# NjuHaoZhang/AMMCNet_AAAI2021

Measured on AMD Instinct MI355X. Metric: frames/sec, 256x256x4 dual-stream clips (twostream forward, inference), higher is better.
Workload: dtype f32-equivalent: (hi,lo) f16 split, 3 fp16 MFMAs per product (v_mfma_f32_32x32x16_f16 in the 4-wave k-half-major kernels, 16x16x32 in the 8-wave / fused-decoder kernels), f32 accumulate; 1 GPU; Ped2 full dual-stream + 2000-slot memory module, batch=16, inference (BASELINE.json configs[1]); batch_per_gpu=16, frame=256x256, n_embed=2000, embed_dim=64, k=2, parallelism=replicas x1 (no collective)

## Files before the change

ammcnet_aaai2021_amd/csrc/conv_outc_s16.hip:

```cpp
#include "ammc_common.h"
#include <hip/hip_fp16.h>
#include <stdio.h>
#include <stdlib.h>

namespace ammc_s16 {

typedef _Float16 f16x8o __attribute__((ext_vector_type(8)));

constexpr float O_LO_INV = 1.f / 2048.f;
constexpr int O_TH = 8, O_TW = 32, O_HW = O_TW + 2, O_HP = (O_TH + 2) * O_HW;
constexpr int O_APIECES = O_HP * 8;
constexpr int O_NT = 512;
constexpr int O_R = (O_APIECES + O_NT - 1) / O_NT;
constexpr int O_ASTAGE = ((O_APIECES + 63) / 64) * 64 * 4;
constexpr int O_MAXNS = 4;
constexpr int O_TG = O_MAXNS * 256;
constexpr int O_NS = 3;
constexpr int O_MAXCC = 2;
static_assert(O_R == 6, "OUTC_WAIT below knows 0, 2, 6 and 8 outstanding operations");

struct OutcArgs {
  AmmcConvDesc d;
  int tiles_x, tiles_y, ncc, kpad, total, nstore;
};

#define OUTC_WAIT(n)                                                              \
  switch (n) {                                                                    \
    case 0: asm volatile("s_waitcnt vmcnt(0)" ::: "memory"); break;               \
    case 2: asm volatile("s_waitcnt vmcnt(2)" ::: "memory"); break;               \
    case 6: asm volatile("s_waitcnt vmcnt(6)" ::: "memory"); break;               \
    default: asm volatile("s_waitcnt vmcnt(8)" ::: "memory"); break;              \
  }

__global__ __launch_bounds__(O_NT, 1) void conv_outc_s16_kernel(OutcArgs a) {
  extern __shared__ __attribute__((aligned(16))) float smem[];
  float* As = smem;
  float* Fs = smem + O_NS * O_ASTAGE;
  float* Tg = Fs + 9 * O_MAXCC * 128;
  float* Scr = Tg + 2 * O_TG;
  float* Sq = Scr + 256;

  const int tid = threadIdx.x, lane = tid & 63, wave = tid >> 6;
  const int l15 = lane & 15, g4 = lane >> 4;
  const AmmcConvDesc& d = a.d;
  const int G = gridDim.x;
  const int first = ammc_xcd_remap(blockIdx.x, G);
  const int ntile = (a.total - first + G - 1) / G;
  const int U = ntile * a.ncc;

  for (int i = tid; i < 9 * a.ncc * 32; i += O_NT) {
    const int chunk = i >> 5, row = (i >> 3) & 3, q = i & 7;
    int sl = q ^ row;
    sl ^= (sl >> 1) & 1;
    const f32x4 w = *reinterpret_cast<const f32x4*>(d.w + (int64_t)row * a.kpad + chunk * 32 + 4 * sl);
    *reinterpret_cast<f32x4*>(Fs + chunk * 128 + row * 32 + 4 * q) = w;
  }

  const int ns = a.nstore;
  const int64_t ycs = d.y_cs > 0 ? d.y_cs : 1;
  const bool score = d.sq_target != nullptr;

  float sc = 1.f, sh = 0.f;
  if (g4 < ns) {
    if (d.scale) sc = d.scale[g4];
    if (d.shift) sh = d.shift[g4];
  }
  asm volatile("" : "+v"(sc), "+v"(sh));

  int a_off[O_R];
#pragma unroll
  for (int j = 0; j < O_R; ++j) {
    int p = j * O_NT + tid;
    p = p < O_APIECES ? p : O_APIECES - 1;
    const int hp = p >> 3;
    int ls = (p & 7) ^ (hp & 7);
    ls ^= (ls >> 1) & 1;
    const int hy = hp / O_HW;
    const int hx = hp - hy * O_HW;
    a_off[j] = (int)((int64_t)hy * d.x_rs + (int64_t)hx * d.x_ps) + 4 * ls;
  }
#define OUTC_ISSUE(tile_, cc_, stage_)                                                                            \
  {                                                                                                               \
    int sp_ = (tile_);                                                                                            \
    const int tx_ = sp_ % a.tiles_x;                                                                              \
    sp_ /= a.tiles_x;                                                                                             \
    const int ty_ = sp_ % a.tiles_y;                                                                              \
    const int b_ = sp_ / a.tiles_y;                                                                               \
    const float* xp_ = d.x + ((int64_t)b_ * d.x_bs + (int64_t)(ty_ * O_TH) * d.x_rs + (int64_t)(tx_ * O_TW) * d.x_ps) + (cc_) * 32; \
    float* dst_ = As + (stage_) * O_ASTAGE + wave * 256;                                                          \
    _Pragma("unroll") for (int j = 0; j < O_R; ++j)                                                               \
      __builtin_amdgcn_global_load_lds(xp_ + a_off[j], (j * O_NT + wave * 64) * 4 < O_ASTAGE ? dst_ + j * O_NT * 4 : Scr, 16, 0, 0); \
  }
  const int tg_e0 = tid < ns * 256 ? tid : 0, tg_e1 = 512 + tid < ns * 256 ? 512 + tid : 0;
  const int64_t tg_o0 = (tg_e0 >> 8) * ycs + ((tg_e0 >> 5) & 7) * d.y_rs + (tg_e0 & 31) * d.y_ps;
  const int64_t tg_o1 = (tg_e1 >> 8) * ycs + ((tg_e1 >> 5) & 7) * d.y_rs + (tg_e1 & 31) * d.y_ps;
#define OUTC_ISSUE_TG(tile_, buf_)                                                                                \
  {                                                                                                               \
    int sp_ = (tile_);                                                                                            \
    const int tx_ = sp_ % a.tiles_x;                                                                              \
    sp_ /= a.tiles_x;                                                                                             \
    const int ty_ = sp_ % a.tiles_y;                                                                              \
    const int b_ = sp_ / a.tiles_y;                                                                               \
    const float* tp_ = d.sq_target + ((int64_t)b_ * d.y_bs + (int64_t)(ty_ * O_TH) * d.y_rs + (int64_t)(tx_ * O_TW) * d.y_ps); \
    __builtin_amdgcn_global_load_lds(tp_ + tg_o0, wave * 64 < ns * 256 ? Tg + (buf_) * O_TG + wave * 64 : Scr, 4, 0, 0);   \
    __builtin_amdgcn_global_load_lds(tp_ + tg_o1, 512 + wave * 64 < ns * 256 ? Tg + (buf_) * O_TG + 512 + wave * 64 : Scr, 4, 0, 0); \
  }

  int i_tile = first, i_cc = 0, i_stage = 0, issued = 0;
#define OUTC_ISSUE_NEXT()                                         \
  {                                                               \
    OUTC_ISSUE(i_tile, i_cc, i_stage);                            \
    ++issued;                                                     \
    i_stage = i_stage + 1 == O_NS ? 0 : i_stage + 1;              \
    if (++i_cc == a.ncc) i_cc = 0, i_tile += G;                   \
  }
  if (score && a.ncc == 1 && U > 0) OUTC_ISSUE_TG(first, 0);
  if (issued < U) OUTC_ISSUE_NEXT();
  if (issued < U) OUTC_ISSUE_NEXT();

  const int slot_hi = 2 * g4 + (g4 & 1), slot_lo = slot_hi ^ 1;
  const int frow = l15 & 3;
  const float* f_hi = Fs + frow * 32 + ((slot_hi ^ frow) << 2);
  const float* f_lo = Fs + frow * 32 + ((slot_lo ^ frow) << 2);
  const int hpb = wave * O_HW + l15;
  f32x4 acc[2], acx[2];
  acc[0] = acc[1] = acx[0] = acx[1] = f32x4{0.f, 0.f, 0.f, 0.f};
  int c_tile = first, c_cc = 0, c_stage = 0, c_par = 0;
  bool pend = false;
  int pend_b = 0;
  asm volatile("s_waitcnt lgkmcnt(0)" ::: "memory");

  for (int u = 0; u < U; ++u) {
    const int nwait = (u + 1 < U ? O_R : 0) + (pend ? 2 : 0);
    OUTC_WAIT(nwait);
    __builtin_amdgcn_s_barrier();
    asm volatile("" ::: "memory");
    if (pend && score && tid == 0) {
      float s = 0.f;
#pragma unroll
      for (int w = 0; w < 8; ++w) s += Sq[(c_par ^ 1) * 8 + w];
      unsafeAtomicAdd(d.sq_acc + pend_b, s);
    }
    const bool last_cc = c_cc + 1 == a.ncc;
    int sp = c_tile;
    const int tx = sp % a.tiles_x;
    sp /= a.tiles_x;
    const int ty = sp % a.tiles_y;
    const int b = sp / a.tiles_y;
    if (score && u + 1 < U && (a.ncc == 1 || c_cc + 2 == a.ncc)) {
      if (a.ncc == 1) OUTC_ISSUE_TG(c_tile + G, c_par ^ 1) else OUTC_ISSUE_TG(c_tile, c_par);
    }
    if (issued < U) OUTC_ISSUE_NEXT();

    const float* Ac = As + c_stage * O_ASTAGE;
    f16x8o fbh[2], fbl[2], fah[2][2], fal[2][2];
#define OUTC_LOAD(tap_, s_)                                                                   \
  {                                                                                           \
    const int chunk_ = (tap_) * a.ncc + c_cc;                                                 \
    fbh[s_] = *reinterpret_cast<const f16x8o*>(f_hi + chunk_ * 128);                          \
    fbl[s_] = *reinterpret_cast<const f16x8o*>(f_lo + chunk_ * 128);                          \
    _Pragma("unroll") for (int pt = 0; pt < 2; ++pt) {                                        \
      const int hp_ = hpb + 16 * pt + ((tap_) / 3) * O_HW + ((tap_) % 3);                     \
      const float* ap_ = Ac + hp_ * 32;                                                       \
      const int sw_ = hp_ & 7;                                                                \
      fah[s_][pt] = *reinterpret_cast<const f16x8o*>(ap_ + ((slot_hi ^ sw_) << 2));           \
      fal[s_][pt] = *reinterpret_cast<const f16x8o*>(ap_ + ((slot_lo ^ sw_) << 2));           \
    }                                                                                         \
  }
    OUTC_LOAD(0, 0);
#pragma unroll
    for (int tap = 0; tap < 9; ++tap) {
      const int cur = tap & 1;
      if (tap < 8) OUTC_LOAD(tap + 1, cur ^ 1);
      __builtin_amdgcn_sched_barrier(0);
#pragma unroll
      for (int pt = 0; pt < 2; ++pt) acc[pt] = __builtin_amdgcn_mfma_f32_16x16x32_f16(fbh[cur], fah[cur][pt], acc[pt], 0, 0, 0);
#pragma unroll
      for (int pt = 0; pt < 2; ++pt) acx[pt] = __builtin_amdgcn_mfma_f32_16x16x32_f16(fbl[cur], fah[cur][pt], acx[pt], 0, 0, 0);
#pragma unroll
      for (int pt = 0; pt < 2; ++pt) acx[pt] = __builtin_amdgcn_mfma_f32_16x16x32_f16(fbh[cur], fal[cur][pt], acx[pt], 0, 0, 0);
      __builtin_amdgcn_sched_barrier(0);
    }
#undef OUTC_LOAD

    pend = last_cc;
    if (last_cc) {
      const int y = ty * O_TH + wave, x0 = tx * O_TW;
      const int ch = g4 < ns ? g4 : 0;
      float sq0 = 0.f;
#pragma unroll
      for (int pt = 0; pt < 2; ++pt) {
        const f32x4 sum = acc[pt] + acx[pt] * O_LO_INV;
        const float r = g4 == 0 ? sum[0] : (g4 == 1 ? sum[1] : (g4 == 2 ? sum[2] : sum[3]));
        float t = r * sc + sh;
        if (d.act == AMMC_ACT_RELU) t = t > 0.f ? t : 0.f;
        else if (d.act == AMMC_ACT_TANH) t = tanhf(t);
        if (g4 < ns) {
          d.y[(int64_t)b * d.y_bs + (int64_t)y * d.y_rs + (int64_t)(x0 + 16 * pt + l15) * d.y_ps + (int64_t)ch * ycs] = t;
          if (score) {
            const float df = 0.5f * (Tg[c_par * O_TG + ch * 256 + wave * 32 + 16 * pt + l15] - t);
            sq0 += df * df;
          }
        }
        acc[pt] = acx[pt] = f32x4{0.f, 0.f, 0.f, 0.f};
      }
      if (score) {
#pragma unroll
        for (int off = 32; off > 0; off >>= 1) sq0 += __shfl_xor(sq0, off);
        if (lane == 0) Sq[c_par * 8 + wave] = sq0;
        asm volatile("s_waitcnt lgkmcnt(0)" ::: "memory");
      }
      pend_b = b;
    }
    c_stage = c_stage + 1 == O_NS ? 0 : c_stage + 1;
    if (++c_cc == a.ncc) c_cc = 0, c_tile += G, c_par ^= 1;
  }
  if (pend && score) {
    __builtin_amdgcn_s_barrier();
    asm volatile("" ::: "memory");
    if (tid == 0) {
      float s = 0.f;
#pragma unroll
      for (int w = 0; w < 8; ++w) s += Sq[(c_par ^ 1) * 8 + w];
      unsafeAtomicAdd(d.sq_acc + pend_b, s);
    }
  }
#undef OUTC_ISSUE
#undef OUTC_ISSUE_TG
#undef OUTC_ISSUE_NEXT
}

int conv_outc_s16_try(const AmmcConvDesc& d, int kpad, hipStream_t stream, char* label, int label_len) {
  constexpr int OUTC_SKIP = -12345;
  if (!(d.outc_stream ? d.outc_stream - 1 : ammc_opt_outc_stream())) return OUTC_SKIP;
  const int ns = d.n_store > 0 ? d.n_store : d.n;
  if (d.ntaps != 9 || d.up != 1 || d.x_step > 1 || !d.y_f32 || d.n != 32 || ns > O_MAXNS || d.res || d.pool_y) return OUTC_SKIP;
  if (d.cin % 32 || d.cin / 32 > O_MAXCC || d.width % O_TW || d.height % O_TH) return OUTC_SKIP;
  if (d.sq_target && !d.sq_acc) return AMMC_EINVAL;
  OutcArgs a;
  a.d = d;
  a.tiles_x = d.width / O_TW;
  a.tiles_y = d.height / O_TH;
  a.ncc = d.cin / 32;
  a.kpad = kpad;
  a.total = d.batch * a.tiles_y * a.tiles_x;
  a.nstore = ns;
  if (label) {
    snprintf(label, label_len, "conv_outc_s16");
    return AMMC_OK;
  }
  constexpr size_t lds = (size_t)(O_NS * O_ASTAGE + 9 * O_MAXCC * 128 + 2 * O_TG + 256 + 16) * sizeof(float);
  static_assert(lds <= 160 * 1024, "LDS budget");
  hipError_t e = hipFuncSetAttribute(reinterpret_cast<const void*>(conv_outc_s16_kernel),
                                     hipFuncAttributeMaxDynamicSharedMemorySize, (int)lds);
  if (e != hipSuccess) return (int)e;
  const int grid = a.total < 256 ? a.total : 256;
  hipLaunchKernelGGL(conv_outc_s16_kernel, dim3(grid), dim3(O_NT), lds, stream, a);
  return ammc_launch_status();
}

}
```

Baseline: 2480 frames/s.

## Restructure output conv as per-pixel tap-by-channel GEMM with LDS shift-add reduction

Result: no change. 2475 frames/s (median of 2 runs) (-0.2%).

```diff
diff --git a/ammcnet_aaai2021_amd/csrc/conv_outc_s16.hip b/ammcnet_aaai2021_amd/csrc/conv_outc_s16.hip
--- a/ammcnet_aaai2021_amd/csrc/conv_outc_s16.hip
+++ b/ammcnet_aaai2021_amd/csrc/conv_outc_s16.hip
@@ -17,6 +17,12 @@
 constexpr int O_TG = O_MAXNS * 256;
 constexpr int O_NS = 3;
 constexpr int O_MAXCC = 2;
+constexpr int O_PT = (O_HP + 15) / 16;
+constexpr int O_KT = (O_PT + 7) / 8;
+constexpr int O_FROWS = 48;
+constexpr int O_ZS = 32;
+constexpr int O_ZG = O_ZS / 4;
+static_assert(O_HP * O_ZS <= O_ASTAGE, "the partial sums of a tile alias one patch stage");
 static_assert(O_R == 6, "OUTC_WAIT below knows 0, 2, 6 and 8 outstanding operations");
 
 struct OutcArgs {
@@ -32,11 +38,19 @@
     default: asm volatile("s_waitcnt vmcnt(8)" ::: "memory"); break;              \
   }
 
+#define OUTC_LDS_BARRIER()                                      \
+  {                                                             \
+    asm volatile("s_waitcnt lgkmcnt(0)" ::: "memory");          \
+    __builtin_amdgcn_s_barrier();                               \
+    asm volatile("" ::: "memory");                              \
+  }
+
+template <int RT>
 __global__ __launch_bounds__(O_NT, 1) void conv_outc_s16_kernel(OutcArgs a) {
   extern __shared__ __attribute__((aligned(16))) float smem[];
   float* As = smem;
   float* Fs = smem + O_NS * O_ASTAGE;
-  float* Tg = Fs + 9 * O_MAXCC * 128;
+  float* Tg = Fs + O_MAXCC * O_FROWS * 32;
   float* Scr = Tg + 2 * O_TG;
   float* Sq = Scr + 256;
 
@@ -48,15 +62,19 @@
   const int ntile = (a.total - first + G - 1) / G;
   const int U = ntile * a.ncc;
 
-  for (int i = tid; i < 9 * a.ncc * 32; i += O_NT) {
-    const int chunk = i >> 5, row = (i >> 3) & 3, q = i & 7;
-    int sl = q ^ row;
+  const int ns = a.nstore;
+  for (int i = tid; i < a.ncc * RT * 16 * 8; i += O_NT) {
+    const int cc = i / (RT * 16 * 8), row = (i >> 3) % (RT * 16), q = i & 7;
+    int sl = q ^ (row & 7);
     sl ^= (sl >> 1) & 1;
-    const f32x4 w = *reinterpret_cast<const f32x4*>(d.w + (int64_t)row * a.kpad + chunk * 32 + 4 * sl);
-    *reinterpret_cast<f32x4*>(Fs + chunk * 128 + row * 32 + 4 * q) = w;
-  }
-
-  const int ns = a.nstore;
+    f32x4 w = f32x4{0.f, 0.f, 0.f, 0.f};
+    if (row < 9 * ns) {
+      const int tap = row / ns, f = row - tap * ns;
+      w = *reinterpret_cast<const f32x4*>(d.w + (int64_t)f * a.kpad + (tap * a.ncc + cc) * 32 + 4 * sl);
+    }
+    *reinterpret_cast<f32x4*>(Fs + (cc * O_FROWS + row) * 32 + 4 * q) = w;
+  }
+
   const int64_t ycs = d.y_cs > 0 ? d.y_cs : 1;
   const bool score = d.sq_target != nullptr;
 
@@ -119,12 +137,28 @@
   if (issued < U) OUTC_ISSUE_NEXT();
 
   const int slot_hi = 2 * g4 + (g4 & 1), slot_lo = slot_hi ^ 1;
-  const int frow = l15 & 3;
-  const float* f_hi = Fs + frow * 32 + ((slot_hi ^ frow) << 2);
-  const float* f_lo = Fs + frow * 32 + ((slot_lo ^ frow) << 2);
-  const int hpb = wave * O_HW + l15;
-  f32x4 acc[2], acx[2];
-  acc[0] = acc[1] = acx[0] = acx[1] = f32x4{0.f, 0.f, 0.f, 0.f};
+  const int npt = wave + 8 * (O_KT - 1) < O_PT ? O_KT : O_KT - 1;
+  int a_hi[O_KT], a_lo[O_KT], z_off[O_KT];
+#pragma unroll
+  for (int k = 0; k < O_KT; ++k) {
+    const int p = 16 * (wave + 8 * k) + l15;
+    const int pc = p < O_HP ? p : O_HP - 1;
+    a_hi[k] = pc * 32 + ((slot_hi ^ (pc & 7)) << 2);
+    a_lo[k] = pc * 32 + ((slot_lo ^ (pc & 7)) << 2);
+    z_off[k] = p < O_HP ? p * O_ZS : -1;
+  }
+  const float* f_hi = Fs + l15 * 32 + ((slot_hi ^ (l15 & 7)) << 2);
+  const float* f_lo = Fs + l15 * 32 + ((slot_lo ^ (l15 & 7)) << 2);
+  const int npass = (9 * ns + O_ZS - 1) / O_ZS;
+  const int tpp = npass > 1 ? O_ZS / ns : 9;
+  const int zsw = l15 & 7;
+  const bool zflip = (l15 & 8) != 0;
+  const int fch = g4 < ns ? g4 : 0;
+  f32x4 acc[O_KT][RT], acx[O_KT][RT];
+#pragma unroll
+  for (int k = 0; k < O_KT; ++k)
+#pragma unroll
+    for (int rt = 0; rt < RT; ++rt) acc[k][rt] = acx[k][rt] = f32x4{0.f, 0.f, 0.f, 0.f};
   int c_tile = first, c_cc = 0, c_stage = 0, c_par = 0;
   bool pend = false;
   int pend_b = 0;
@@ -153,56 +187,78 @@
     if (issued < U) OUTC_ISSUE_NEXT();
 
     const float* Ac = As + c_stage * O_ASTAGE;
-    f16x8o fbh[2], fbl[2], fah[2][2], fal[2][2];
-#define OUTC_LOAD(tap_, s_)                                                                   \
-  {                                                                                           \
-    const int chunk_ = (tap_) * a.ncc + c_cc;                                                 \
-    fbh[s_] = *reinterpret_cast<const f16x8o*>(f_hi + chunk_ * 128);                          \
-    fbl[s_] = *reinterpret_cast<const f16x8o*>(f_lo + chunk_ * 128);                          \
-    _Pragma("unroll") for (int pt = 0; pt < 2; ++pt) {                                        \
-      const int hp_ = hpb + 16 * pt + ((tap_) / 3) * O_HW + ((tap_) % 3);                     \
-      const float* ap_ = Ac + hp_ * 32;                                                       \
-      const int sw_ = hp_ & 7;                                                                \
-      fah[s_][pt] = *reinterpret_cast<const f16x8o*>(ap_ + ((slot_hi ^ sw_) << 2));           \
-      fal[s_][pt] = *reinterpret_cast<const f16x8o*>(ap_ + ((slot_lo ^ sw_) << 2));           \
-    }                                                                                         \
-  }
-    OUTC_LOAD(0, 0);
-#pragma unroll
-    for (int tap = 0; tap < 9; ++tap) {
-      const int cur = tap & 1;
-      if (tap < 8) OUTC_LOAD(tap + 1, cur ^ 1);
-      __builtin_amdgcn_sched_barrier(0);
-#pragma unroll
-      for (int pt = 0; pt < 2; ++pt) acc[pt] = __builtin_amdgcn_mfma_f32_16x16x32_f16(fbh[cur], fah[cur][pt], acc[pt], 0, 0, 0);
-#pragma unroll
-      for (int pt = 0; pt < 2; ++pt) acx[pt] = __builtin_amdgcn_mfma_f32_16x16x32_f16(fbl[cur], fah[cur][pt], acx[pt], 0, 0, 0);
-#pragma unroll
-      for (int pt = 0; pt < 2; ++pt) acx[pt] = __builtin_amdgcn_mfma_f32_16x16x32_f16(fbh[cur], fal[cur][pt], acx[pt], 0, 0, 0);
-      __builtin_amdgcn_sched_barrier(0);
-    }
-#undef OUTC_LOAD
+    f16x8o fbh[RT], fbl[RT], fah[O_KT], fal[O_KT];
+#pragma unroll
+    for (int rt = 0; rt < RT; ++rt) {
+      fbh[rt] = *reinterpret_cast<const f16x8o*>(f_hi + (c_cc * O_FROWS + rt * 16) * 32);
+      fbl[rt] = *reinterpret_cast<const f16x8o*>(f_lo + (c_cc * O_FROWS + rt * 16) * 32);
+    }
+#pragma unroll
+    for (int k = 0; k < O_KT; ++k) {
+      fah[k] = *reinterpret_cast<const f16x8o*>(Ac + a_hi[k]);
+      fal[k] = *reinterpret_cast<const f16x8o*>(Ac + a_lo[k]);
+    }
+#pragma unroll
+    for (int k = 0; k < O_KT; ++k) {
+      if (k < npt) {
+#pragma unroll
+        for (int rt = 0; rt < RT; ++rt) acc[k][rt] = __builtin_amdgcn_mfma_f32_16x16x32_f16(fbh[rt], fah[k], acc[k][rt], 0, 0, 0);
+#pragma unroll
+        for (int rt = 0; rt < RT; ++rt) acx[k][rt] = __builtin_amdgcn_mfma_f32_16x16x32_f16(fbl[rt], fah[k], acx[k][rt], 0, 0, 0);
+#pragma unroll
+        for (int rt = 0; rt < RT; ++rt) acx[k][rt] = __builtin_amdgcn_mfma_f32_16x16x32_f16(fbh[rt], fal[k], acx[k][rt], 0, 0, 0);
+      }
+    }
 
     pend = last_cc;
     if (last_cc) {
+      float* Z = As + c_stage * O_ASTAGE;
       const int y = ty * O_TH + wave, x0 = tx * O_TW;
-      const int ch = g4 < ns ? g4 : 0;
+      float rs[2] = {0.f, 0.f};
+      OUTC_LDS_BARRIER();
+      for (int pass = 0; pass < npass; ++pass) {
+        if (pass) OUTC_LDS_BARRIER();
+#pragma unroll
+        for (int k = 0; k < O_KT; ++k) {
+#pragma unroll
+          for (int rt = 0; rt < RT; ++rt) {
+            const int grp = 4 * rt + g4, q = grp - O_ZG * pass;
+            if (k < npt && z_off[k] >= 0 && 4 * grp < 9 * ns && q >= 0 && q < O_ZG) {
+              const f32x4 v = acc[k][rt] + acx[k][rt] * O_LO_INV;
+              *reinterpret_cast<f32x4*>(Z + z_off[k] + ((q ^ zsw) << 2)) = zflip ? f32x4{v[2], v[3], v[0], v[1]} : v;
+            }
+          }
+        }
+        OUTC_LDS_BARRIER();
+#pragma unroll
+        for (int tap = 0; tap < 9; ++tap) {
+          if (tap >= tpp * pass && tap < tpp * (pass + 1)) {
+            const int pix = (wave + tap / 3) * O_HW + l15 + tap % 3;
+            const int row = tap * ns + g4 - O_ZS * pass;
+            const float* zp = Z + pix * O_ZS + ((((row >> 2) ^ pix) & 7) << 2) + ((row ^ (pix >> 2)) & 2) + (row & 1);
+            rs[0] += zp[0];
+            rs[1] += zp[16 * O_ZS];
+          }
+        }
+      }
+#pragma unroll
+      for (int k = 0; k < O_KT; ++k)
+#pragma unroll
+        for (int rt = 0; rt < RT; ++rt) acc[k][rt] = acx[k][rt] = f32x4{0.f, 0.f, 0.f, 0.f};
+
       float sq0 = 0.f;
 #pragma unroll
       for (int pt = 0; pt < 2; ++pt) {
-        const f32x4 sum = acc[pt] + acx[pt] * O_LO_INV;
-        const float r = g4 == 0 ? sum[0] : (g4 == 1 ? sum[1] : (g4 == 2 ? sum[2] : sum[3]));
-        float t = r * sc + sh;
+        float t = rs[pt] * sc + sh;
         if (d.act == AMMC_ACT_RELU) t = t > 0.f ? t : 0.f;
         else if (d.act == AMMC_ACT_TANH) t = tanhf(t);
         if (g4 < ns) {
-          d.y[(int64_t)b * d.y_bs + (int64_t)y * d.y_rs + (int64_t)(x0 + 16 * pt + l15) * d.y_ps + (int64_t)ch * ycs] = t;
+          d.y[(int64_t)b * d.y_bs + (int64_t)y * d.y_rs + (int64_t)(x0 + 16 * pt + l15) * d.y_ps + (int64_t)fch * ycs] = t;
           if (score) {
-            const float df = 0.5f * (Tg[c_par * O_TG + ch * 256 + wave * 32 + 16 * pt + l15] - t);
+            const float df = 0.5f * (Tg[c_par * O_TG + fch * 256 + wave * 32 + 16 * pt + l15] - t);
             sq0 += df * df;
           }
         }
-        acc[pt] = acx[pt] = f32x4{0.f, 0.f, 0.f, 0.f};
       }
       if (score) {
 #pragma unroll
@@ -249,13 +305,13 @@
     snprintf(label, label_len, "conv_outc_s16");
     return AMMC_OK;
   }
-  constexpr size_t lds = (size_t)(O_NS * O_ASTAGE + 9 * O_MAXCC * 128 + 2 * O_TG + 256 + 16) * sizeof(float);
+  constexpr size_t lds = (size_t)(O_NS * O_ASTAGE + O_MAXCC * O_FROWS * 32 + 2 * O_TG + 256 + 16) * sizeof(float);
   static_assert(lds <= 160 * 1024, "LDS budget");
-  hipError_t e = hipFuncSetAttribute(reinterpret_cast<const void*>(conv_outc_s16_kernel),
-                                     hipFuncAttributeMaxDynamicSharedMemorySize, (int)lds);
+  auto* kernel = 9 * ns <= 32 ? conv_outc_s16_kernel<2> : conv_outc_s16_kernel<3>;
+  hipError_t e = hipFuncSetAttribute(reinterpret_cast<const void*>(kernel), hipFuncAttributeMaxDynamicSharedMemorySize, (int)lds);
   if (e != hipSuccess) return (int)e;
   const int grid = a.total < 256 ? a.total : 256;
-  hipLaunchKernelGGL(conv_outc_s16_kernel, dim3(grid), dim3(O_NT), lds, stream, a);
+  hipLaunchKernelGGL(kernel, dim3(grid), dim3(O_NT), lds, stream, a);
   return ammc_launch_status();
 }
 
```
